# pkubioinformatics/nanoreviser

Hardware: AMD Instinct MI355X
Metric: bases revised/sec (whole node) (higher is better)
Workload: dtype f32 via scaled 2xf16 split (f32 accumulate)

## Files before the change

nanoreviser_amd/csrc/nrv_api.hip:

```cpp
#include "../../include/nanorev.h"
#include "nrv_kernels.h"
#include "nrv_tailfit.h"
#include "nrv_block.h"

#include <algorithm>
#include <cmath>
#include <cstdio>
#include <cstdlib>
#include <cstring>
#include <string>
#include <chrono>
#include <vector>

using namespace nrv;

#ifdef NRV_DEV_FAST
#define NRV_ACT1(...)
#else
#define NRV_ACT1(...) __VA_ARGS__
#endif

namespace {

thread_local std::string g_create_error = "";
// ... 3626 lines not shown
  if (p && n > 0) HIPCHK(h, hipMemcpyAsync(p, h->fit.d_p, (size_t)n * C * 4, hipMemcpyDeviceToHost, h->stream));
  return fit_state_get(h, model, stats);
}

int nrv_fit_params(nrv_handle* h, int model, float* params, int64_t* t) {
  static const char* who = "nrv_fit_params";
  const int rc = fit_enter(h, who);
  if (rc) return rc;
  if (model != 0 && model != 1) return fit_refuse(h, who, "model must be 0 or 1");
  if (!h->fit.m[model].begun) return fit_refuse(h, who, "no fit in progress for this model (call nrv_fit_begin first)");
  HIPCHK(h, hipStreamSynchronize(h->stream));
  if (params) HIPCHK(h, hipMemcpy(params, h->fit.m[model].d_par, (size_t)fit_params_n(h, model) * 4, hipMemcpyDeviceToHost));
  if (t) *t = h->fit.m[model].t;
  return NRV_OK;
}

int nrv_saturated(nrv_handle* h, int64_t* pending, int64_t* reruns) {
  int rc = check_handle(h);
  if (rc) return rc;
  unsigned v = 0;
  HIPCHK(h, hipStreamSynchronize(h->stream));
  HIPCHK(h, hipMemcpy(&v, h->d_sat + 2, sizeof(unsigned), hipMemcpyDeviceToHost));
  if (v) HIPCHK(h, hipMemset(h->d_sat + 2, 0, sizeof(unsigned)));
  if (pending) *pending = (int64_t)v;
  if (reruns) *reruns = h->sat_reruns;
  return NRV_OK;
}

int nrv_prof_enable(nrv_handle* h, int on) {
  int rc = check_handle(h);
  if (rc) return rc;
  if ((rc = prof_collect(h))) return rc;
  h->prof = (on == 2 || on == 3) ? on : (on != 0);
  h->prof_tick = 0;
  return NRV_OK;
}

int nrv_prof_read(nrv_handle* h, double* ms_total, int64_t* launches) {
  int rc = check_handle(h);
  if (rc) return rc;
  if ((rc = prof_collect(h))) return rc;
  for (int k = 0; k < NRV_N_KERNELS; ++k) {
    if (ms_total) ms_total[k] = h->prof_ms[k];
    if (launches) launches[k] = h->prof_n[k];
    h->prof_ms[k] = 0;
    h->prof_n[k] = 0;
  }
  return NRV_OK;
}

int nrv_prof_overhead(nrv_handle* h, double* us) {
  int rc = check_handle(h);
  if (rc) return rc;
  if (!us) { h->err = "nrv_prof_overhead: null output"; return NRV_E_INVALID; }
  constexpr int N = 64;
  struct Events {
    hipEvent_t ev[2 * N];
    int n = 0;
    ~Events() { for (int i = 0; i < n; ++i) (void)hipEventDestroy(ev[i]); }
  } E;
  for (; E.n < 2 * N; ++E.n) HIPCHK(h, hipEventCreate(&E.ev[E.n]));
  HIPCHK(h, hipStreamSynchronize(h->stream));
  for (int i = 0; i < 2 * N; ++i) HIPCHK(h, hipEventRecord(E.ev[i], h->stream));
  HIPCHK(h, hipStreamSynchronize(h->stream));
  double tot = 0;
  for (int i = 0; i < N; ++i) {
    float ms = 0.f;
    HIPCHK(h, hipEventElapsedTime(&ms, E.ev[2 * i], E.ev[2 * i + 1]));
    tot += ms;
  }
  *us = tot / N * 1e3;
  return NRV_OK;
}

#if NRV_STAMP
int nrv_exp_only_stage(int k) {
  g_only_stage = k;
  return 0;
}
int nrv_exp_stamps(void* dst, size_t bytes) {
  if (bytes > sizeof(nrv::nrv_stamp_buf)) bytes = sizeof(nrv::nrv_stamp_buf);
  return hipMemcpyFromSymbol(dst, HIP_SYMBOL(nrv::nrv_stamp_buf), bytes, 0, hipMemcpyDeviceToHost) == hipSuccess ? (int)0 : -1;
}
#endif

const char* nrv_kernel_name(int slot) {
  static const char* names[NRV_N_KERNELS] = {"cnn_kernel", "lstm1_kernel 6->16", "lstm2 32->64", "lstm3 192->128",
                                             "lstm4 256->64", "head_mlp+head_final"};
  return (slot >= 0 && slot < NRV_N_KERNELS) ? names[slot] : "";
}

const char* nrv_last_error(nrv_handle* h) { return h ? h->err.c_str() : g_create_error.c_str(); }
int nrv_backend(nrv_handle* h) { (void)h; return NRV_BACKEND_HIP; }
int nrv_device_count(void) {
  int n = 0;
  return hipGetDeviceCount(&n) == hipSuccess && n > 0 ? n : 0;
}
int nrv_window(nrv_handle* h) { return h ? h->T : NRV_E_INVALID; }

}
```

nanoreviser_amd/csrc/nrv_cnn_r.h:

```cpp
#pragma once
#include "nrv_common.h"
#include "nrv_lstm_f16x2s.h"
#include "nrv_lstm1.h"

namespace nrv {

struct CnnRConsts {
  float w1[24];
  float b1[8];
  float s1[8], h1[8];
};
struct CnnRModelParams {
  const void* w2frag;
  const float* ep;
  const void* dfrag;
  const float* dbias;
  float* out;
};
struct CnnRArgs {
  CnnRModelParams m[2];
  CnnRConsts k[2];
  const float* signal;
  int T, n_rows, n_tiles;
  unsigned* sat;
  Lstm1ModelParams l1[2];
  int l1_T, l1_rows;
};

constexpr int kCnnRWaves = 8;
constexpr int kCnnRL1Waves = 4;
constexpr int kCnnRThreads = 64 * (kCnnRWaves + kCnnRL1Waves);
constexpr float kCnnRImgScale = 64.0f;
constexpr float kCnnRDenseDescale = 1.0f / 1024.0f;

typedef float f32x2r __attribute__((ext_vector_type(2)));
typedef _Float16 f16x2r __attribute__((ext_vector_type(2)));
typedef _Float16 f16x4r __attribute__((ext_vector_type(4)));
typedef __attribute__((address_space(3))) float lds_f32r;

constexpr int kCnnRRing = 12, kCnnRSlot = 2 * 16 * 8, kCnnRC1Wave = kCnnRRing * kCnnRSlot;

template <int ACT>
__global__ void __launch_bounds__(kCnnRThreads) cnn_r_kernel(const CnnRArgs args) {
  constexpr int NKS = 13;
  __shared__ __attribute__((aligned(16))) float wd_s[NKS * 4 * 2 * 256];
  __shared__ __attribute__((aligned(16))) _Float16 c1_s[kCnnRWaves * kCnnRC1Wave + 2 * kCnnRSlot];
  __shared__ __attribute__((aligned(16))) float l1h_s[kCnnRL1Waves][16 * 16 + 16];
  const CnnRModelParams& P = args.m[blockIdx.y];
  const CnnRConsts& K = args.k[blockIdx.y];
  const int T = args.T;
  const int wave = __builtin_amdgcn_readfirstlane(threadIdx.x >> 6);
  const int lane = threadIdx.x & 63;
  const int n = lane & 15, q = lane >> 4;

  const __amdgpu_buffer_rsrc_t wrs = make_rsrc(P.dfrag, NKS * 8 * 1024);
  for (int base = 0; base < NKS * 8 * 64; base += 8 * kCnnRThreads) {
    f32x4 v[8];
#pragma unroll
    for (int j = 0; j < 8; ++j) v[j] = buf_load16(wrs, (unsigned)(base + j * kCnnRThreads + threadIdx.x) * 16, 0);
#pragma unroll
    for (int j = 0; j < 8; ++j)
      if (base + j * kCnnRThreads + threadIdx.x < NKS * 8 * 64) ((f32x4*)wd_s)[base + j * kCnnRThreads + threadIdx.x] = v[j];
  }
  static_assert((kCnnRWaves * kCnnRC1Wave + 2 * kCnnRSlot) % 8 == 0, "ring image in 16-byte pieces");
  for (int i = threadIdx.x; i < (kCnnRWaves * kCnnRC1Wave + 2 * kCnnRSlot) / 8; i += kCnnRThreads) ((f32x4*)c1_s)[i] = f32x4{0.f, 0.f, 0.f, 0.f};
  __syncthreads();

  if (wave >= kCnnRWaves) {
    const int nu = 2 * ((args.l1_rows + 15) / 16);
    for (int idx = blockIdx.x * kCnnRL1Waves + (wave - kCnnRWaves); idx < nu; idx += gridDim.x * kCnnRL1Waves)
      lstm1_unit<ACT, true>(args.l1[blockIdx.y], args.l1_T, args.l1_rows, idx & 1, idx >> 1, lane, l1h_s[wave - kCnnRWaves]);
    return;
  }

  typedef __attribute__((address_space(3))) _Float16 lds_h;
  typedef __attribute__((address_space(3))) f16x8 lds_h8;
  lds_h* const c1 = (lds_h*)c1_s + wave * kCnnRC1Wave;
  const f16x8 a2_hi = *(const f16x8*)((const char*)P.w2frag + lane * 16);
  const f16x8 a2_lo = *(const f16x8*)((const char*)P.w2frag + 1024 + lane * 16);
  const int c0 = 4 * (q & 1);
  const f32x4 binit = *(const f32x4*)(P.ep + c0);
  const f32x4 k1 = *(const f32x4*)(P.ep + 8 + c0);
  const f32x4 k2 = *(const f32x4*)(P.ep + 16 + c0);
  f32x4 dbias[4];
#pragma unroll
  for (int mt = 0; mt < 4; ++mt) dbias[mt] = *(const f32x4*)(P.dbias + 16 * mt + 4 * q);
  const float* wd = wd_s + lane * 4;
  bool bad = false;
#define w1v K.w1
#define b1v K.b1
#define s1v K.s1
#define h1v K.h1
  auto relu_acc = [](float x) __attribute__((always_inline)) { return __builtin_amdgcn_fmed3f(x, 0.f, 3.0e38f); };
  float m1; asm("s_mov_b32 %0, 0xbf800000" : "=s"(m1));
#define NRV_LO(x, h) __builtin_fmaf((float)(h), m1, (x))
  lds_h* const rq = c1 + q * kCnnRSlot + n * 8;
  lds_h* const rq9 = c1 + ((9 + q) % kCnnRRing) * kCnnRSlot + n * 8;
  lds_h* const rq11 = c1 + ((11 + q) % kCnnRRing) * kCnnRSlot + n * 8;
  lds_h* const zslot = (lds_h*)c1_s + kCnnRWaves * kCnnRC1Wave + n * 8;
  auto slot_c = [&](int C) __attribute__((always_inline)) {
    const int cm = ((C % kCnnRRing) + kCnnRRing) % kCnnRRing;
    return cm == 9 ? rq9 : cm == 11 ? rq11 : rq + cm * kCnnRSlot;
  };

  const int n_units = 2 * args.n_tiles;
  float xmax = 0.f;
  auto conv1_store = [&](lds_h* d, float xm, float xc, float xp) __attribute__((always_inline)) {
    xmax = __builtin_amdgcn_fmed3f(__builtin_fabsf(xc), xmax, 3.0e38f);
    float c[8];
#pragma unroll
    for (int o = 0; o < 8; ++o) {
      float tt = b1v[o];
      tt = __builtin_fmaf(xm, w1v[0 * 8 + o], tt);
      tt = __builtin_fmaf(xc, w1v[1 * 8 + o], tt);
      tt = __builtin_fmaf(xp, w1v[2 * 8 + o], tt);
      tt = __builtin_fmaxf(tt, 0.f);
      c[o] = __builtin_fmaf(tt, s1v[o], h1v[o]);
    }
    f16x8 hi, lo;
#pragma unroll
    for (int o = 0; o < 8; o += 2) {
      const f16x2r hp = __builtin_convertvector(f32x2r{c[o], c[o + 1]}, f16x2r);
      hi[o] = hp[0]; hi[o + 1] = hp[1];
      const f16x2r lp = __builtin_convertvector(f32x2r{NRV_LO(c[o], hp[0]), NRV_LO(c[o + 1], hp[1])}, f16x2r);
      lo[o] = lp[0]; lo[o + 1] = lp[1];
    }
    *(lds_h8*)d = hi;
    *(lds_h8*)(d + 16 * 8) = lo;
  };


  for (int u = blockIdx.x + gridDim.x * wave; u < n_units; u += gridDim.x * kCnnRWaves) {
    const int b = u >> 1, sub = u & 1;
    const int wt = b / T, t = b % T;
    const int row = 16 * sub + n;
    const bool rok = wt * 32 + row < args.n_rows;
    const size_t ev0 = (size_t)wt * 32 * T + t, left = ((size_t)args.n_rows * T - ev0) * (kSig * 4);
    const __amdgpu_buffer_rsrc_t rs = make_rsrc(args.signal + ev0 * kSig, left < 0x7fffffffu ? (unsigned)left : 0x7fffffffu);
    constexpr unsigned kOut = 0x80000000u;
    const unsigned xq = rok ? (unsigned)(row * T * kSig + q) * 4u : kOut;
    const unsigned xh = rok ? (unsigned)(row * T * kSig + (q >> 1)) * 4u : kOut;
    auto ldq = [&](int C) __attribute__((always_inline)) {
      if (C >= kSig) return 0.f;
      return buf_load4(rs, (C + 3 < kSig || q < kSig - C ? xq : kOut) + 4u * C, 0);
    };
    auto ldh = [&](int C) __attribute__((always_inline)) {
      if (C >= kSig) return 0.f;
      return buf_load4(rs, (C + 1 < kSig || (q >> 1) < kSig - C ? xh : kOut) + 4u * C, 0);
    };
// ... 120 lines not shown
```

nanoreviser_amd/csrc/nrv_head_f16x2.h:

```cpp
#pragma once
#include "nrv_head.h"
#include "nrv_lstm_f16x2.h"

namespace nrv {

struct HeadH2ModelParams {
  const void* wsplit;
  const float* bias;
  const float* in;
  const float* featw;
  const float* featb;
  const float* outw;
  const float* outb;
  float* prob;
  int8_t* argmax;
  float c12, c23, c3o;
  int n_class;
};
struct HeadH2Args {
  HeadH2ModelParams m[2];
  int T;
  int n_rows;
  int n_tiles;
};

constexpr int kHeadH2Threads = 512;

__global__ void __launch_bounds__(kHeadH2Threads) head_h2_kernel(const HeadH2Args args) {
  constexpr int NT = kHeadH2Threads, NW = NT / 64;
  constexpr int NFRAG = 84;
  constexpr int TMAX = kHeadMaxT;
  __shared__ __attribute__((aligned(16))) unsigned short wl[NFRAG * 512];
  __shared__ __attribute__((aligned(16))) float bl[192];
  __shared__ __attribute__((aligned(16))) float mo[TMAX * 32 * 8];
  __shared__ __attribute__((aligned(16))) float fw8[16 * TMAX * 8];
  __shared__ float featv[32 * 17];
  __shared__ float logit[32 * 8];
  __shared__ float tl[16 + 8 + 16 * 8];
  const HeadH2ModelParams& P = args.m[blockIdx.y];
  const int T = args.T;
  const int tid = threadIdx.x, lane = tid & 63, half = lane >> 5, l31 = lane & 31;
  const int wave = __builtin_amdgcn_readfirstlane(tid >> 6);
  {
    const __amdgpu_buffer_rsrc_t srs = make_rsrc(P.wsplit, NFRAG * 1024);
    for (int base = 0; base < NFRAG * 64; base += 8 * NT) {
      f32x4 v[8];
#pragma unroll
      for (int j = 0; j < 8; ++j) v[j] = buf_load16(srs, (unsigned)(base + j * NT + tid) * 16, 0);
#pragma unroll
      for (int j = 0; j < 8; ++j)
        if (base + j * NT + tid < NFRAG * 64) ((f32x4*)wl)[base + j * NT + tid] = v[j];
    }
  }
  if (tid < 192) bl[tid] = P.bias[tid];
  {
    const int C0 = P.n_class;
    if (tid >= 256 && tid < 272) tl[tid - 256] = P.featb[tid - 256];
    else if (tid >= 272 && tid < 280) tl[tid - 256] = tid - 272 < C0 ? P.outb[tid - 272] : 0.f;
    else if (tid >= 320 && tid < 320 + 16 * C0) tl[24 + tid - 320] = P.outw[tid - 320];
  }
  for (int i = tid; i < 16 * T * 2; i += NT) ((f32x4*)fw8)[i] = ((const f32x4*)P.featw)[i];
  const unsigned av = l31 * 16 + half * 512;
  auto load_x = [&](int u, f32x4 (&x)[8][2]) __attribute__((always_inline)) {
    const __amdgpu_buffer_rsrc_t ars = make_rsrc(P.in + (size_t)u * 32 * 128, 32 * 128 * 4);
#pragma unroll
    for (int kb = 0; kb < 8; ++kb) {
      x[kb][0] = buf_load16(ars, av, kb * 2048);
      x[kb][1] = buf_load16(ars, av, kb * 2048 + 1024);
    }
  };
  f32x4 x[8][2];
  if (wave < T && (int)blockIdx.x < args.n_tiles) load_x(blockIdx.x * T + wave, x);
  __syncthreads();

  const float m1 = neg_one_opaque();
  constexpr int PW[3] = {1, 0, 0}, PX[3] = {0, 1, 0};
  auto frag = [&](int f) __attribute__((always_inline)) { return *(const f16x8*)(wl + f * 512 + lane * 8); };
  auto bias_tile = [&](int off) __attribute__((always_inline)) {
    f32x16 z;
#pragma unroll
    for (int q = 0; q < 4; ++q) {
      const f32x4 v = *(const f32x4*)(bl + off + 8 * q + 4 * half);
#pragma unroll
      for (int j = 0; j < 4; ++j) z[4 * q + j] = v[j];
    }
    return z;
  };
  auto relu_split = [&](const f32x16& z, int base, float c) __attribute__((always_inline)) {
    f32x4 lo, hi;
#pragma unroll
    for (int j = 0; j < 4; ++j) {
      lo[j] = relu_nan(z[base + j] * c);
      hi[j] = relu_nan(z[base + 4 + j] * c);
    }
    return split2(lo, hi, m1);
  };

  for (int tile = blockIdx.x; tile < args.n_tiles; tile += gridDim.x) {
    if (wave < T && tile != (int)blockIdx.x) load_x(tile * T + wave, x);
    for (int t = wave; t < T; t += NW) {
      f32x16 acc[4];
#pragma unroll
      for (int mt = 0; mt < 4; ++mt) acc[mt] = bias_tile(mt * 32);
#pragma unroll
      for (int kb = 0; kb < 8; ++kb) {
        f16x8 w[4][2];
#pragma unroll
        for (int mt = 0; mt < 4; ++mt)
#pragma unroll
          for (int tm = 0; tm < 2; ++tm) w[mt][tm] = frag((mt * 8 + kb) * 2 + tm);
        __builtin_amdgcn_sched_barrier(0);
        const f16x8 xs[2] = {__builtin_bit_cast(f16x8, x[kb][0]), __builtin_bit_cast(f16x8, x[kb][1])};
#pragma unroll
        for (int pr = 0; pr < 3; ++pr)
#pragma unroll
          for (int mt = 0; mt < 4; ++mt) acc[mt] = mfma_f16(w[mt][PW[pr]], xs[PX[pr]], acc[mt]);
        __builtin_amdgcn_sched_barrier(0);
      }
      if (t + NW < T) load_x(tile * T + t + NW, x);
      f32x16 a2[2];
      a2[0] = bias_tile(128);
      a2[1] = splat16(0.f);
#pragma unroll
      for (int kb = 0; kb < 8; ++kb) {
        const Split2 s2 = relu_split(acc[kb >> 1], (kb & 1) * 8, P.c12);
        const f16x8 w2[2] = {frag(64 + kb * 2), frag(64 + kb * 2 + 1)};
#pragma unroll
        for (int pr = 0; pr < 3; ++pr) a2[kb & 1] = mfma_f16(w2[PW[pr]], s2.t[PX[pr]], a2[kb & 1]);
        __builtin_amdgcn_sched_barrier(0);
      }
      f32x16 h2;
#pragma unroll
      for (int i = 0; i < 16; ++i) h2[i] = a2[0][i] + a2[1][i];
      f32x16 a3 = bias_tile(160);
#pragma unroll
      for (int kb = 0; kb < 2; ++kb) {
        const Split2 s3 = relu_split(h2, kb * 8, P.c23);
        const f16x8 w3[2] = {frag(80 + kb * 2), frag(80 + kb * 2 + 1)};
#pragma unroll
        for (int pr = 0; pr < 3; ++pr) a3 = mfma_f16(w3[PW[pr]], s3.t[PX[pr]], a3);
      }
      f32x4 o;
#pragma unroll
      for (int j = 0; j < 4; ++j) o[j] = relu_nan(a3[j] * P.c3o);
      *(f32x4*)(mo + (t * 32 + l31) * 8 + 4 * half) = o;
    }
    __syncthreads();

    for (int it = tid; it < 32 * 16; it += NT) {
      const int r = it >> 4, f = it & 15;
      float v = tl[f];
      for (int t = 0; t < T; ++t) {
        const f32x4 x0 = *(const f32x4*)(mo + (t * 32 + r) * 8), x1 = *(const f32x4*)(mo + (t * 32 + r) * 8 + 4);
        const f32x4 w0 = *(const f32x4*)(fw8 + (f * T + t) * 8), w1 = *(const f32x4*)(fw8 + (f * T + t) * 8 + 4);
        v = __builtin_fmaf(x0[0], w0[0], v);
        v = __builtin_fmaf(x0[1], w0[1], v);
// ... 41 lines not shown
```

nanoreviser_amd/csrc/nrv_kernels.h:

```cpp
#pragma once
#include "nrv_common.h"
#include "nrv_cnn.h"
#include "nrv_lstm1.h"
#include "nrv_lstm_f32.h"
#include "nrv_lstm_bf16x3.h"
#include "nrv_lstm_f16x2.h"
#include "nrv_lstm_f16x2s.h"
#include "nrv_lstm_f16x2w.h"
#include "nrv_lstm2_u.h"
#include "nrv_cnn_r.h"
#include "nrv_head.h"
#include "nrv_head_f16x2.h"
#include "nrv_segment.h"
#include "nrv_stats.h"
#include "nrv_merge.h"
#include "nrv_report.h"
#include "nrv_edits.h"
#include "nrv_pack.h"
#include "nrv_profile.h"
#include "nrv_trim.h"
#include "nrv_align.h"
#include "nrv_errclass.h"
#include "nrv_infix.h"
#include "nrv_labels.h"
#include "nrv_score.h"
```

nanoreviser_amd/csrc/nrv_lstm2_u.h:

```cpp
#pragma once
#include "nrv_lstm_f16x2s.h"

namespace nrv {

constexpr int kL2uThreads = 512;

struct Lstm2TModelParams {
  const void* wfrag;
  const float* bias;
  const float* in;
  float* out;
  float descale;
};
struct Lstm2TArgs {
  Lstm2TModelParams m[2];
  int T;
  int n_rows;
};

typedef float f32x2 __attribute__((ext_vector_type(2)));
typedef _Float16 f16x2 __attribute__((ext_vector_type(2)));

constexpr int kL2tWFrags = 3 * 16 * 2;

__device__ __forceinline__ void lstm2_t_stage(const Lstm2TModelParams& P, const int dir, float* wl, float* bl,
                                              const int tid, const int nthreads) {
  const __amdgpu_buffer_rsrc_t wrs = make_rsrc((const char*)P.wfrag + (size_t)dir * kL2tWFrags * 1024, kL2tWFrags * 1024);
  for (int base = 0; base < kL2tWFrags * 64; base += 8 * nthreads) {
    f32x4 v[8];
#pragma unroll
    for (int j = 0; j < 8; ++j) v[j] = buf_load16(wrs, (unsigned)(base + j * nthreads + tid) * 16, 0);
#pragma unroll
    for (int j = 0; j < 8; ++j)
      if (base + j * nthreads + tid < kL2tWFrags * 64) ((f32x4*)wl)[base + j * nthreads + tid] = v[j];
  }
  const f32x4* bsrc = (const f32x4*)(P.bias + (size_t)dir * 16 * 256);
  for (int i = tid; i < 16 * 64; i += nthreads) ((f32x4*)bl)[i] = bsrc[i];
}


template <int ACT>
__device__ __forceinline__ void lstm2_u_unit(const Lstm2TModelParams& P, const int T, const int dir, const int rb,
                                             const int lane, const int hf, const float* wl, const float* bl, f32x4* hx) {
  constexpr int NR = 4, LEAD = 3;
  const int n = lane & 15, q = lane >> 4;
  const int tile = rb >> 1, trow = 16 * (rb & 1) + n;
  const float dsc = P.descale, dsc02 = 0.2f * dsc, dsc2 = 2.885390081777927f * dsc;
  const __amdgpu_buffer_rsrc_t xrs = make_rsrc(P.in + (size_t)tile * T * 8 * 128, (unsigned)T * 8 * 512);
  const unsigned xv = (unsigned)((4 * (q >> 1) + (q & 1)) * 512 + trow * 16);
  auto t_of = [&](int s) __attribute__((always_inline)) { const int sc = s < T ? s : T - 1; return dir ? (T - 1 - sc) : sc; };
  struct XFrag { f32x4 hi, lo; };
  auto load_x = [&](int s) __attribute__((always_inline)) {
    XFrag x;
    const unsigned so = (unsigned)t_of(s) * 8 * 512;
    x.lo = __builtin_bit_cast(f32x4, __builtin_amdgcn_raw_buffer_load_b128(xrs, xv + 1024, so, 0));
    x.hi = __builtin_bit_cast(f32x4, __builtin_amdgcn_raw_buffer_load_b128(xrs, xv, so, 0));
    return x;
  };
  float* const obase = P.out + ((size_t)tile * T * 32 + (dir * 4) * 4 + (q >> 1)) * 128 + trow * 4 + (q & 1) * 2 + (size_t)hf * 2 * 4 * 128;
  const float* const wlh = wl + hf * 2 * 2 * 256 + lane * 4;
  const float* const blh = bl + hf * 2 * 256 + lane * 4;

  struct WPair { f32x4 hi, lo; };
  WPair wr[NR];
  auto frag_of = [&](int ci) __attribute__((always_inline)) {
    if (ci < 16) { const int u = ci >> 3, g = (ci >> 1) & 3, kb = 1 + (ci & 1); return ((kb * 16) + g * 4 + u) * 2; }
    const int u = (ci - 16) >> 2, g = (ci - 16) & 3;
    return (g * 4 + u) * 2;
  };
  auto load_w = [&](int ci) __attribute__((always_inline)) {
    const int f = frag_of(ci);
    wr[ci % NR].lo = *(const f32x4*)(wlh + (f + 1) * 256);
    wr[ci % NR].hi = *(const f32x4*)(wlh + f * 256);
  };

  f32x4 Z[8];
  float c[8];
  f16x8 hB[2][2];
  f16x8 hN[2];
#pragma unroll
  for (int i = 0; i < 8; ++i) c[i] = 0.f;

  constexpr int GST = 13;
  struct GateSt { float zi, zf, zg, zo, cp, p, t; };
  GateSt gsr;
  float hv[4];
  auto gate_stage = [&](int u, int r, int st, int t_out) __attribute__((always_inline)) {
    const int e = 4 * u + r;
    GateSt& gs = gsr;
    if (st == 0) { gs.zi = Z[0 + u][r]; gs.zf = Z[2 + u][r]; gs.cp = c[e]; }
    else if (st == 1) { gs.zg = Z[4 + u][r]; gs.zo = Z[6 + u][r]; }
    else if (st == 2) {
      if constexpr (ACT == 0) {
        gs.zi = __builtin_fminf(__builtin_fmaxf(__builtin_fmaf(gs.zi, dsc02, 0.5f), 0.0f), 1.0f);
        gs.zf = __builtin_fminf(__builtin_fmaxf(__builtin_fmaf(gs.zf, dsc02, 0.5f), 0.0f), 1.0f);
      } else {
        gs.zi = sigmoid_exact(gs.zi * dsc);
        gs.zf = sigmoid_exact(gs.zf * dsc);
      }
    } else if (st == 3) {
      if constexpr (ACT == 0) gs.zo = __builtin_fminf(__builtin_fmaxf(__builtin_fmaf(gs.zo, dsc02, 0.5f), 0.0f), 1.0f);
      else gs.zo = sigmoid_exact(gs.zo * dsc);
      gs.zg = gs.zg * dsc2;
    } else if (st == 4) gs.zg = __builtin_amdgcn_exp2f(gs.zg);
    else if (st == 5) gs.t = __builtin_amdgcn_rcpf(gs.zg + 1.0f);
    else if (st == 6) gs.p = gs.zi * __builtin_fmaf(gs.t, -2.0f, 1.0f);
    else if (st == 7) {
      const float cn = __builtin_fmaf(gs.zf, gs.cp, gs.p);
      c[e] = cn;
      gs.zg = cn * 2.885390081777927f;
    } else if (st == 8) gs.zg = __builtin_amdgcn_exp2f(gs.zg);
    else if (st == 9) gs.t = __builtin_amdgcn_rcpf(gs.zg + 1.0f);
    else if (st == 10) hv[r] = gs.zo * __builtin_fmaf(gs.t, -2.0f * kHScale, kHScale);
    else if (st == 11) {
      if (r & 1) {
        const f16x2 hp = __builtin_convertvector(f32x2{hv[r - 1], hv[r]}, f16x2);
        hN[0][4 * u + r - 1] = hp[0];
        hN[0][4 * u + r] = hp[1];
      }
    } else {
// ... 49 lines not shown
    const f16x8 xb[2] = {__builtin_bit_cast(f16x8, x.hi), __builtin_bit_cast(f16x8, x.lo)};
#pragma unroll
    for (int g = 0; g < 4; ++g) Z[g * 2] = *(const f32x4*)(blh + (g * 4) * 256);
#pragma unroll
    for (int k = 0; k < 8; ++k) {
      const int ci = 16 + k, u = k >> 2, g = k & 3;
      load_w(ci + LEAD < 24 ? ci + LEAD : ci + LEAD - 24);
      if (k == 4) {
#pragma unroll
        for (int gg = 0; gg < 4; ++gg) Z[gg * 2 + 1] = *(const f32x4*)(blh + (gg * 4 + 1) * 256);
      }
      __builtin_amdgcn_sched_barrier(0);
#pragma unroll
      for (int pr = 0; pr < 3; ++pr) {
        const f16x8 a = __builtin_bit_cast(f16x8, PA[pr] ? wr[ci % NR].lo : wr[ci % NR].hi);
        Z[g * 2 + u] = mfma16_f16(a, xb[PB[pr]], Z[g * 2 + u]);
        if constexpr (GATES1) {
          const int tk = k * 3 + pr;
          if (tk < 12) {
#pragma unroll
            for (int pc = (tk * NGP) / 12; pc < ((tk + 1) * NGP) / 12; ++pc) gate_piece(1, pc, t_out);
          }
        }
        __builtin_amdgcn_sched_barrier(0);
      }
    }
  };
  auto exchange = [&](int p) __attribute__((always_inline)) {
    f32x4* const img = hx + p * 4 * 64 + lane;
    img[(hf * 2 + 0) * 64] = __builtin_bit_cast(f32x4, hN[0]);
    img[(hf * 2 + 1) * 64] = __builtin_bit_cast(f32x4, hN[1]);
    __syncthreads();
#pragma unroll
    for (int kb = 0; kb < 2; ++kb)
#pragma unroll
      for (int tm = 0; tm < 2; ++tm) hB[kb][tm] = __builtin_bit_cast(f16x8, img[(kb * 2 + tm) * 64]);
  };

  XFrag xn = load_x(1);
  {
    const XFrag x0 = load_x(0);
#pragma unroll
    for (int i = 0; i < LEAD; ++i) load_w(16 + i);
    in_phase(std::false_type{}, x0, 0);
#pragma unroll
    for (int i = 0; i < LEAD; ++i) load_w(16 + i);
  }
  {
    const int t0 = t_of(0);
    gates_plain(0, t0);
    if (T > 1) {
      const XFrag x = xn;
      xn = load_x(2);
      in_phase(std::true_type{}, x, t0);
      exchange(0);
    } else {
      gates_plain(1, t0);
    }
  }
#pragma unroll 1
  for (int s = 1; s < T; ++s) {
    const int t = t_of(s);
    rec_phase(t);
    if (s + 1 < T) {
      const XFrag x = xn;
      xn = load_x(s + 2);
      in_phase(std::true_type{}, x, t);
      exchange(s & 1);
    } else {
      gates_plain(1, t);
    }
  }
}

template <int ACT>
__global__ void __launch_bounds__(kL2uThreads) lstm2_u_kernel(const Lstm2TArgs args) {
  __shared__ __attribute__((aligned(16))) float wl[kL2tWFrags * 256];
  __shared__ __attribute__((aligned(16))) float bl[16 * 256];
  __shared__ __attribute__((aligned(16))) f32x4 hx[4 * 2 * 4 * 64];
  const Lstm2TModelParams& P = args.m[blockIdx.z];
  const int lane = threadIdx.x & 63;
  const int wave = __builtin_amdgcn_readfirstlane(threadIdx.x >> 6);
  const int chain = wave & 3, hf = wave >> 2;
  lstm2_t_stage(P, blockIdx.y, wl, bl, threadIdx.x, kL2uThreads);
  __syncthreads();
  lstm2_u_unit<ACT>(P, args.T, blockIdx.y, blockIdx.x * 4 + chain, lane, hf, wl, bl, hx + chain * 2 * 4 * 64);
}

}
```

nanoreviser_amd/csrc/nrv_lstm_f16x2s.h:

```cpp
#pragma once
#include "nrv_lstm_f16x2.h"

namespace nrv {

#ifndef NRV_STAMP
#define NRV_STAMP 0
#endif
#if NRV_STAMP
constexpr int kStampSlots = 32, kStampSteps = 15, kStampWaves = 4, kStampBlocks = 256;
__device__ unsigned long long nrv_stamp_buf[2][kStampBlocks][kStampWaves][kStampSteps][kStampSlots];
#define NRV_STAMP_AT(slot)                                                                                   \
  do {                                                                                                       \
    __builtin_amdgcn_sched_barrier(0);                                                                       \
    unsigned long long t_;                                                                                   \
    asm volatile("s_memtime %0\n\ts_waitcnt lgkmcnt(0)" : "=s"(t_)::"memory");                               \
    stamp_lds[(wave * kStampSteps + stamp_step) * kStampSlots + (slot)] = t_;                                \
    __builtin_amdgcn_sched_barrier(0);                                                                       \
  } while (0)
#else
#define NRV_STAMP_AT(slot) do { } while (0)
#endif

__device__ __forceinline__ f32x4 mfma16_f16(const f16x8& a, const f16x8& b, f32x4 c) {
  return __builtin_amdgcn_mfma_f32_16x16x32_f16(a, b, c, 0, 0, 0);
}

template <int KQ0, int KQ1, int H, int R, int WR, int UH, int ACT, int NBG, int NA, int KBL = 0, bool RAW = false>
__global__ void __launch_bounds__(64 * (H / (16 * UH)) * WR)
lstm_h2s_kernel(const LstmH2Args args) {
  constexpr int NG = H / (16 * UH);
  constexpr int KK0 = KQ0 / 8, KK1 = KQ1 / 8, KK_IN = KK0 + KK1, KK_REC = H / 32, KK = KK_IN + KK_REC;
  constexpr int RT = 2 * R;
  constexpr int EPK = 4 * UH, TPE = 3 * RT;
  constexpr int ROWS = 32 * R * WR;
  constexpr int GS = ROWS * 8 + 8;
  constexpr int TERM = (H / 8) * GS;
  constexpr int HBUF = TERM;
  constexpr int NTHREADS = 64 * NG * WR;
  constexpr int LBG = NBG - 1, LA = NA - 1;
  static_assert(KQ0 % 8 == 0 && KQ1 % 8 == 0 && H % 32 == 0 && H % (16 * UH) == 0, "K must come in blocks of 32");
  static_assert((EPK * KK) % NBG == 0 && (EPK * KK_IN) % NBG == 0 && KK % NA == 0 && KK_IN % NA == 0,
                "ring sizes must divide the block counts");
  static_assert(LA >= 1 && LA <= KK_IN && LA <= KK_REC && LBG <= EPK * KK_REC, "leads must stay inside a phase");

  constexpr int NE = UH * RT * 4;
  constexpr bool CLDS = NE > 32;
  __shared__ __attribute__((aligned(16))) float hbuf[2 * HBUF];
  __shared__ __attribute__((aligned(16))) float bnl[2 * H];
  __shared__ float cl[CLDS ? NE * NTHREADS : 1];
  __shared__ __attribute__((aligned(16))) float wl[KBL > 0 ? NG * WR * KBL * EPK * 512 : 4];

  const int lane = threadIdx.x & 63;
  const int wave = __builtin_amdgcn_readfirstlane(threadIdx.x >> 6);
#if NRV_STAMP
  __shared__ unsigned long long stamp_lds[kStampWaves * kStampSteps * kStampSlots];
  int stamp_step = 0;
  for (int i = threadIdx.x; i < kStampWaves * kStampSteps * kStampSlots; i += 64 * (H / (16 * UH)) * WR) stamp_lds[i] = 0;
  unsigned long long stamp_rt0;
  asm volatile("s_memrealtime %0\n\ts_waitcnt lgkmcnt(0)" : "=s"(stamp_rt0)::"memory");
#endif
  const int hg = wave % NG, wr = wave / NG;
  const int l15 = lane & 15, kq = lane >> 4;
  const LstmBlock blk = lstm_block();
  if (blk.rowblk >= args.n_blk) return;
  const int dir = blk.dir;
  const LstmH2ModelParams& P = args.m[blk.model];
  const int T = args.T;
  const int row0 = blk.rowblk * ROWS + wr * (32 * R);
  const int lrow0 = wr * (32 * R);

  const __amdgpu_buffer_rsrc_t wrs = make_rsrc(
      (const char*)P.wsplit + ((size_t)(dir * NG + hg) * KK) * (EPK * 2 * 1024), KK * EPK * 2 * 1024);
  const unsigned wlane = lane * 16;
  const float* bp = P.bias + (size_t)(dir * NG + hg) * 4 * (16 * UH) + l15;
  const float dsc = P.descale, dsc02 = 0.2f * dsc, dsc2 = 2.885390081777927f * dsc;
  float kI[UH], kF[UH], kO[UH], kG[UH], bzI[UH], bzF[UH], bzO[UH];
#pragma unroll
  for (int uh = 0; uh < UH; ++uh) {
    const float bi = bp[0 * 16 * UH + 16 * uh] * dsc, bf = bp[1 * 16 * UH + 16 * uh] * dsc,
                bg = bp[2 * 16 * UH + 16 * uh] * dsc, bo = bp[3 * 16 * UH + 16 * uh] * dsc;
    kI[uh] = __builtin_fmaf(bi, 0.2f, 0.5f); kF[uh] = __builtin_fmaf(bf, 0.2f, 0.5f);
    kO[uh] = __builtin_fmaf(bo, 0.2f, 0.5f); kG[uh] = bg * 2.885390081777927f;
    bzI[uh] = bi; bzF[uh] = bf; bzO[uh] = bo;
  }
  const int u0 = hg * 16 * UH + l15;
  const int hw_off = (u0 >> 3) * GS + (lrow0 + 4 * kq) * 8 + (u0 & 7);
  const int hp_off = kq * GS + (lrow0 + l15) * 8;

  float* const wlw = wl + (wave * KBL * EPK) * 512 + lane * 4;
  if constexpr (KBL > 0) {
#pragma unroll 1
    for (int e0 = 0; e0 < KBL * EPK; e0 += 4) {
      f32x4 v[8];
#pragma unroll
      for (int j = 0; j < 8; ++j)
        if (e0 + j / 2 < KBL * EPK) v[j] = buf_load16(wrs, wlane, ((e0 + j / 2) * 2 + (j & 1)) * 1024);
#pragma unroll
      for (int j = 0; j < 8; ++j)
        if (e0 + j / 2 < KBL * EPK) *(f32x4*)(wlw + ((e0 + j / 2) * 2 + (j & 1)) * 256) = v[j];
    }
  }
  for (int i = threadIdx.x; i < 2 * H; i += NTHREADS)
    bnl[i] = i < H ? P.out_scale[dir * H + i] : P.out_shift[dir * H + i - H];
  for (int i = threadIdx.x; i < HBUF; i += NTHREADS) hbuf[i] = 0.f;
  float c[CLDS ? 1 : NE];
  if constexpr (CLDS) {
#pragma unroll
    for (int i = 0; i < NE; ++i) cl[i * NTHREADS + threadIdx.x] = 0.f;
  } else {
#pragma unroll
    for (int i = 0; i < NE; ++i) c[i] = 0.f;
  }
  __syncthreads();

  struct ABase {
    __amdgpu_buffer_rsrc_t r0[R], r1[R];
    unsigned v0[R][2], v1[R][2];
  };
  auto mk_base = [&](int s) __attribute__((always_inline)) {
    const int sc = s < T ? s : T - 1;
    const int t = dir ? (T - 1 - sc) : sc;
    ABase ab;
#pragma unroll
    for (int r = 0; r < R; ++r) {
      ab.r0[r] = make_rsrc(P.in0.ubase(row0 + r * 32, t), 0xffffffffu);
      if constexpr (KQ1 > 0) ab.r1[r] = make_rsrc(P.in1.ubase(row0 + r * 32, t), 0xffffffffu);
      else ab.r1[r] = ab.r0[r];
#pragma unroll
      for (int sub = 0; sub < 2; ++sub) {
        ab.v0[r][sub] = (P.in0.voff(row0 + r * 32, t, l15 + 16 * sub, kq & 1) + (kq >> 1) * 512) * 4;
        if constexpr (KQ1 > 0) ab.v1[r][sub] = (P.in1.voff(row0 + r * 32, t, l15 + 16 * sub, kq & 1) + (kq >> 1) * 512) * 4;
        else ab.v1[r][sub] = 0;
      }
    }
    return ab;
  };
  struct BReg { f16x8 t[2]; };
  struct AReg { f32x4 v[2]; };
  BReg b[NBG];
  AReg a[NA][RT];
  auto loadB = [&](int e, BReg& bb) __attribute__((always_inline)) {
    if (KBL > 0 && e < KBL * EPK) {
      bb.t[0] = __builtin_bit_cast(f16x8, *(const f32x4*)(wlw + (e * 2) * 256));
      bb.t[1] = __builtin_bit_cast(f16x8, *(const f32x4*)(wlw + (e * 2 + 1) * 256));
    } else {
      bb.t[0] = __builtin_bit_cast(f16x8, buf_load16(wrs, wlane, (e * 2) * 1024));
      bb.t[1] = __builtin_bit_cast(f16x8, buf_load16(wrs, wlane, (e * 2 + 1) * 1024));
    }
  };
  auto loadA_in = [&](const ABase& ab, int kk, int rt, AReg& d) __attribute__((always_inline)) {
    const int r = rt >> 1, sub = rt & 1;
    if (KQ1 == 0 || kk < KK0) {
      d.v[1] = buf_load16(ab.r0[r], ab.v0[r][sub], kk * 4096 + 1024);
      d.v[0] = buf_load16(ab.r0[r], ab.v0[r][sub], kk * 4096);
    } else {
      d.v[1] = buf_load16(ab.r1[r], ab.v1[r][sub], (kk - KK0) * 4096 + 1024);
      d.v[0] = buf_load16(ab.r1[r], ab.v1[r][sub], (kk - KK0) * 4096);
    }
  };
  auto loadA_rec = [&](const _Float16* hp, int kkr, int rt, AReg& d) __attribute__((always_inline)) {
    const _Float16* qh = hp + kkr * 4 * GS + rt * 128;
    d.v[1] = *(const f32x4*)(qh + TERM);
    d.v[0] = *(const f32x4*)(qh);
  };
  auto loadB1 = [&](int e, int term, BReg& bb) __attribute__((always_inline)) {
    if (KBL > 0 && e < KBL * EPK) bb.t[term] = __builtin_bit_cast(f16x8, *(const f32x4*)(wlw + (e * 2 + term) * 256));
    else bb.t[term] = __builtin_bit_cast(f16x8, buf_load16(wrs, wlane, (e * 2 + term) * 1024));
  };
  auto loadA_in1 = [&](const ABase& ab, int kk, int rt, int term, AReg& d) __attribute__((always_inline)) {
    const int r = rt >> 1, sub = rt & 1;
    if (KQ1 == 0 || kk < KK0) d.v[term] = buf_load16(ab.r0[r], ab.v0[r][sub], kk * 4096 + term * 1024);
    else d.v[term] = buf_load16(ab.r1[r], ab.v1[r][sub], (kk - KK0) * 4096 + term * 1024);
  };
  auto loadA_rec1 = [&](const _Float16* hp, int kkr, int rt, int term, AReg& d) __attribute__((always_inline)) {
    d.v[term] = *(const f32x4*)(hp + kkr * 4 * GS + rt * 128 + term * TERM);
  };
  constexpr int APPE = (2 * RT + EPK - 1) / EPK;
  static_assert(4 + APPE <= 3 * RT, "fragment pieces must fit behind an entry's products");
  constexpr int PA[3] = {0, 1, 0}, PB[3] = {1, 0, 0};

  constexpr int GST = 14;
  struct GateSt { float zi, zf, zg, zo, cp, p, hv, t; _Float16 hh, hl; };
  auto gate_stage = [&](GateSt& g, const f32x4 (&Z)[4][UH][RT], _Float16* hw, int e, int st) __attribute__((always_inline)) {
    const int uh = e / (RT * 4), rt = (e / 4) % RT, reg = e % 4;
    if (st == 0) {
      g.zi = Z[0][uh][rt][reg]; g.zf = Z[1][uh][rt][reg];
      if constexpr (CLDS) g.cp = cl[e * NTHREADS + threadIdx.x];
      else g.cp = c[e];
    } else if (st == 1) {
      g.zg = Z[2][uh][rt][reg]; g.zo = Z[3][uh][rt][reg];
    } else if (st == 2) {
      if constexpr (ACT == 0) {
        g.zi = __builtin_fminf(__builtin_fmaxf(__builtin_fmaf(g.zi, dsc02, kI[uh]), 0.0f), 1.0f);
        g.zf = __builtin_fminf(__builtin_fmaxf(__builtin_fmaf(g.zf, dsc02, kF[uh]), 0.0f), 1.0f);
      } else {
        g.zi = sigmoid_exact(__builtin_fmaf(g.zi, dsc, bzI[uh]));
// ... 243 lines not shown
```

Measured before the change: 12.43 million.

## Stage weight fragments into LDS via direct global-to-LDS loads with rotation

After: 12.52 million, median of 6. No clear change (+0.8%).

```diff
diff --git a/nanoreviser_amd/csrc/nrv_api.hip b/nanoreviser_amd/csrc/nrv_api.hip
--- a/nanoreviser_amd/csrc/nrv_api.hip
+++ b/nanoreviser_amd/csrc/nrv_api.hip
@@ -3732,6 +3732,10 @@
   if (bytes > sizeof(nrv::nrv_stamp_buf)) bytes = sizeof(nrv::nrv_stamp_buf);
   return hipMemcpyFromSymbol(dst, HIP_SYMBOL(nrv::nrv_stamp_buf), bytes, 0, hipMemcpyDeviceToHost) == hipSuccess ? (int)0 : -1;
 }
+int nrv_exp_stage_stamps(void* dst, size_t bytes) {
+  if (bytes > sizeof(nrv::nrv_stage_stamp_buf)) bytes = sizeof(nrv::nrv_stage_stamp_buf);
+  return hipMemcpyFromSymbol(dst, HIP_SYMBOL(nrv::nrv_stage_stamp_buf), bytes, 0, hipMemcpyDeviceToHost) == hipSuccess ? (int)0 : -1;
+}
 #endif
 
 const char* nrv_kernel_name(int slot) {
diff --git a/nanoreviser_amd/csrc/nrv_cnn_r.h b/nanoreviser_amd/csrc/nrv_cnn_r.h
--- a/nanoreviser_amd/csrc/nrv_cnn_r.h
+++ b/nanoreviser_amd/csrc/nrv_cnn_r.h
@@ -2,6 +2,7 @@
 #include "nrv_common.h"
 #include "nrv_lstm_f16x2s.h"
 #include "nrv_lstm1.h"
+#include "nrv_stage.h"
 
 namespace nrv {
 
@@ -53,18 +54,12 @@
   const int lane = threadIdx.x & 63;
   const int n = lane & 15, q = lane >> 4;
 
-  const __amdgpu_buffer_rsrc_t wrs = make_rsrc(P.dfrag, NKS * 8 * 1024);
-  for (int base = 0; base < NKS * 8 * 64; base += 8 * kCnnRThreads) {
-    f32x4 v[8];
-#pragma unroll
-    for (int j = 0; j < 8; ++j) v[j] = buf_load16(wrs, (unsigned)(base + j * kCnnRThreads + threadIdx.x) * 16, 0);
-#pragma unroll
-    for (int j = 0; j < 8; ++j)
-      if (base + j * kCnnRThreads + threadIdx.x < NKS * 8 * 64) ((f32x4*)wd_s)[base + j * kCnnRThreads + threadIdx.x] = v[j];
-  }
+  NRV_STAGE_ENTRY();
+  stage_frags_lds(P.dfrag, wd_s, NKS * 8, wave, kCnnRWaves + kCnnRL1Waves, lane, 0);
   static_assert((kCnnRWaves * kCnnRC1Wave + 2 * kCnnRSlot) % 8 == 0, "ring image in 16-byte pieces");
   for (int i = threadIdx.x; i < (kCnnRWaves * kCnnRC1Wave + 2 * kCnnRSlot) / 8; i += kCnnRThreads) ((f32x4*)c1_s)[i] = f32x4{0.f, 0.f, 0.f, 0.f};
   __syncthreads();
+  NRV_STAGE_DONE(0, blockIdx.x + gridDim.x * blockIdx.y);
 
   if (wave >= kCnnRWaves) {
     const int nu = 2 * ((args.l1_rows + 15) / 16);
diff --git a/nanoreviser_amd/csrc/nrv_head_f16x2.h b/nanoreviser_amd/csrc/nrv_head_f16x2.h
--- a/nanoreviser_amd/csrc/nrv_head_f16x2.h
+++ b/nanoreviser_amd/csrc/nrv_head_f16x2.h
@@ -1,6 +1,7 @@
 #pragma once
 #include "nrv_head.h"
 #include "nrv_lstm_f16x2.h"
+#include "nrv_stage.h"
 
 namespace nrv {
 
@@ -41,6 +42,7 @@
   const int T = args.T;
   const int tid = threadIdx.x, lane = tid & 63, half = lane >> 5, l31 = lane & 31;
   const int wave = __builtin_amdgcn_readfirstlane(tid >> 6);
+  NRV_STAGE_ENTRY();
   {
     const __amdgpu_buffer_rsrc_t srs = make_rsrc(P.wsplit, NFRAG * 1024);
     for (int base = 0; base < NFRAG * 64; base += 8 * NT) {
@@ -72,6 +74,7 @@
   f32x4 x[8][2];
   if (wave < T && (int)blockIdx.x < args.n_tiles) load_x(blockIdx.x * T + wave, x);
   __syncthreads();
+  NRV_STAGE_DONE(3, blockIdx.x + gridDim.x * blockIdx.y);
 
   const float m1 = neg_one_opaque();
   constexpr int PW[3] = {1, 0, 0}, PX[3] = {0, 1, 0};
diff --git a/nanoreviser_amd/csrc/nrv_kernels.h b/nanoreviser_amd/csrc/nrv_kernels.h
--- a/nanoreviser_amd/csrc/nrv_kernels.h
+++ b/nanoreviser_amd/csrc/nrv_kernels.h
@@ -1,5 +1,6 @@
 #pragma once
 #include "nrv_common.h"
+#include "nrv_stage.h"
 #include "nrv_cnn.h"
 #include "nrv_lstm1.h"
 #include "nrv_lstm_f32.h"
diff --git a/nanoreviser_amd/csrc/nrv_lstm2_u.h b/nanoreviser_amd/csrc/nrv_lstm2_u.h
--- a/nanoreviser_amd/csrc/nrv_lstm2_u.h
+++ b/nanoreviser_amd/csrc/nrv_lstm2_u.h
@@ -1,5 +1,6 @@
 #pragma once
 #include "nrv_lstm_f16x2s.h"
+#include "nrv_stage.h"
 
 namespace nrv {
 
@@ -25,17 +26,9 @@
 
 __device__ __forceinline__ void lstm2_t_stage(const Lstm2TModelParams& P, const int dir, float* wl, float* bl,
                                               const int tid, const int nthreads) {
-  const __amdgpu_buffer_rsrc_t wrs = make_rsrc((const char*)P.wfrag + (size_t)dir * kL2tWFrags * 1024, kL2tWFrags * 1024);
-  for (int base = 0; base < kL2tWFrags * 64; base += 8 * nthreads) {
-    f32x4 v[8];
-#pragma unroll
-    for (int j = 0; j < 8; ++j) v[j] = buf_load16(wrs, (unsigned)(base + j * nthreads + tid) * 16, 0);
-#pragma unroll
-    for (int j = 0; j < 8; ++j)
-      if (base + j * nthreads + tid < kL2tWFrags * 64) ((f32x4*)wl)[base + j * nthreads + tid] = v[j];
-  }
-  const f32x4* bsrc = (const f32x4*)(P.bias + (size_t)dir * 16 * 256);
-  for (int i = tid; i < 16 * 64; i += nthreads) ((f32x4*)bl)[i] = bsrc[i];
+  const int wave = __builtin_amdgcn_readfirstlane(tid >> 6);
+  stage_frags_lds((const char*)P.wfrag + (size_t)dir * kL2tWFrags * 1024, wl, kL2tWFrags, wave, nthreads / 64, tid & 63, 0);
+  stage_frags_lds(P.bias + (size_t)dir * 16 * 256, bl, 16, wave, nthreads / 64, tid & 63, 0);
 }
 
 
@@ -251,8 +244,10 @@
   const int lane = threadIdx.x & 63;
   const int wave = __builtin_amdgcn_readfirstlane(threadIdx.x >> 6);
   const int chain = wave & 3, hf = wave >> 2;
+  NRV_STAGE_ENTRY();
   lstm2_t_stage(P, blockIdx.y, wl, bl, threadIdx.x, kL2uThreads);
   __syncthreads();
+  NRV_STAGE_DONE(1, blockIdx.x + gridDim.x * (blockIdx.y + gridDim.y * blockIdx.z));
   lstm2_u_unit<ACT>(P, args.T, blockIdx.y, blockIdx.x * 4 + chain, lane, hf, wl, bl, hx + chain * 2 * 4 * 64);
 }
 
diff --git a/nanoreviser_amd/csrc/nrv_lstm_f16x2s.h b/nanoreviser_amd/csrc/nrv_lstm_f16x2s.h
--- a/nanoreviser_amd/csrc/nrv_lstm_f16x2s.h
+++ b/nanoreviser_amd/csrc/nrv_lstm_f16x2s.h
@@ -1,5 +1,6 @@
 #pragma once
 #include "nrv_lstm_f16x2.h"
+#include "nrv_stage.h"
 
 namespace nrv {
 
@@ -59,6 +60,7 @@
   unsigned long long stamp_rt0;
   asm volatile("s_memrealtime %0\n\ts_waitcnt lgkmcnt(0)" : "=s"(stamp_rt0)::"memory");
 #endif
+  NRV_STAGE_ENTRY();
   const int hg = wave % NG, wr = wave / NG;
   const int l15 = lane & 15, kq = lane >> 4;
   const LstmBlock blk = lstm_block();
@@ -88,18 +90,9 @@
   const int hp_off = kq * GS + (lrow0 + l15) * 8;
 
   float* const wlw = wl + (wave * KBL * EPK) * 512 + lane * 4;
-  if constexpr (KBL > 0) {
-#pragma unroll 1
-    for (int e0 = 0; e0 < KBL * EPK; e0 += 4) {
-      f32x4 v[8];
-#pragma unroll
-      for (int j = 0; j < 8; ++j)
-        if (e0 + j / 2 < KBL * EPK) v[j] = buf_load16(wrs, wlane, ((e0 + j / 2) * 2 + (j & 1)) * 1024);
-#pragma unroll
-      for (int j = 0; j < 8; ++j)
-        if (e0 + j / 2 < KBL * EPK) *(f32x4*)(wlw + ((e0 + j / 2) * 2 + (j & 1)) * 256) = v[j];
-    }
-  }
+  if constexpr (KBL > 0)
+    stage_frags_lds((const char*)P.wsplit + ((size_t)(dir * NG + hg) * KK) * (EPK * 2 * 1024), wl + (wave * KBL * EPK) * 512,
+                    KBL * EPK * 2, 0, 1, lane, stage_rot(blockIdx.x, 3, KBL * EPK * 2));
   for (int i = threadIdx.x; i < 2 * H; i += NTHREADS)
     bnl[i] = i < H ? P.out_scale[dir * H + i] : P.out_shift[dir * H + i - H];
   for (int i = threadIdx.x; i < HBUF; i += NTHREADS) hbuf[i] = 0.f;
@@ -112,6 +105,7 @@
     for (int i = 0; i < NE; ++i) c[i] = 0.f;
   }
   __syncthreads();
+  if constexpr (KBL > 0) NRV_STAGE_DONE(2, blockIdx.x);
 
   struct ABase {
     __amdgpu_buffer_rsrc_t r0[R], r1[R];
diff --git a/nanoreviser_amd/csrc/nrv_stage.h b/nanoreviser_amd/csrc/nrv_stage.h
--- /dev/null
+++ b/nanoreviser_amd/csrc/nrv_stage.h
@@ -0,0 +1,55 @@
+#pragma once
+
+#if defined(__HIPCC__)
+#include "nrv_common.h"
+#define NRV_STAGE_HD __host__ __device__
+#else
+#define NRV_STAGE_HD
+#endif
+
+namespace nrv {
+
+NRV_STAGE_HD constexpr int frag_at(int k, int rot, int n_frags) { return (k + rot) % n_frags; }
+
+NRV_STAGE_HD constexpr int stage_rot(int id, int stride, int n_frags) { return ((id / 8) * stride) % n_frags; }
+
+#if defined(__HIPCC__)
+__device__ __forceinline__ void stage_frags_lds(const void* src, float* lds, int n_frags, int wave, int n_waves, int lane, int rot) {
+  typedef __attribute__((address_space(1))) char gchar;
+  typedef __attribute__((address_space(3))) char lchar;
+  gchar* const g = (gchar*)const_cast<void*>(src) + lane * 16;
+  lchar* const l = (lchar*)lds;
+  for (int k = wave; k < n_frags; k += n_waves) {
+    const int f = frag_at(k, rot, n_frags);
+    __builtin_amdgcn_global_load_lds(g + f * 1024, l + f * 1024, 16, 0, 0);
+  }
+}
+
+#ifndef NRV_STAMP
+#define NRV_STAMP 0
+#endif
+#if NRV_STAMP
+constexpr int kStageStampKernels = 4, kStageStampBlocks = 256;
+__device__ unsigned long long nrv_stage_stamp_buf[kStageStampKernels][kStageStampBlocks][2];
+#define NRV_STAGE_ENTRY()                                                                                    \
+  unsigned long long stage_t0_;                                                                              \
+  asm volatile("s_memtime %0\n\ts_waitcnt lgkmcnt(0)" : "=s"(stage_t0_)::"memory");                          \
+  __builtin_amdgcn_sched_barrier(0)
+#define NRV_STAGE_DONE(kernel, id)                                                                           \
+  do {                                                                                                       \
+    __builtin_amdgcn_sched_barrier(0);                                                                       \
+    unsigned long long t1_;                                                                                  \
+    asm volatile("s_memtime %0\n\ts_waitcnt lgkmcnt(0)" : "=s"(t1_)::"memory");                              \
+    if (threadIdx.x == 0 && (id) < kStageStampBlocks) {                                                      \
+      nrv_stage_stamp_buf[kernel][id][0] = stage_t0_;                                                        \
+      nrv_stage_stamp_buf[kernel][id][1] = t1_;                                                              \
+    }                                                                                                        \
+    __builtin_amdgcn_sched_barrier(0);                                                                       \
+  } while (0)
+#else
+#define NRV_STAGE_ENTRY() do { } while (0)
+#define NRV_STAGE_DONE(kernel, id) do { } while (0)
+#endif
+#endif
+
+}
```
